# sleep3r/Diffusion-Handwriting-Generation.pytorch

Measured on AMD Instinct MI355X. Metric: stroke-points/sec reverse-sampled (T=60, L=488), higher is better.
Workload: dtype bf16; 1 GPU; configs[1]: batch=64 prompts/GPU, T=60, L=488, Lt=30, d_model=128/192/256, num_layers=2, diffusion_mode=new, random-init weights; global_batch=64, seq_len=488, parallelism=batch-shard x1 (no collectives)

## Files before the change

diffusion-handwriting-generation.pytorch_amd/build.py:

```python
from __future__ import annotations

import os
import subprocess
import sys
from concurrent.futures import ThreadPoolExecutor

HERE = os.path.dirname(os.path.abspath(__file__))
CSRC = os.path.join(HERE, "csrc")
LIB = os.path.join(HERE, "libdhw_hip.so")
SOURCES = ["train/sgemm_f32.hip", "train/sgemm_bf16.hip", "train/sgemm_group.hip", "convblock.hip", "ragged/convblock_ragged.hip", "enclayer.hip",
           "ragged/enclayer_ragged.hip", "policy/convblock_policy.hip", "policy/enclayer_policy.hip", "gemm.hip", "ragged/gemm_ragged.hip", "ragged/attn_ragged.hip", "persist.hip", "attn.hip", "misc.hip", "style.hip", "textside.hip",
           "train.hip", "train/sgemm_launch.hip", "train/elementwise.hip", "train/film_table.hip", "train/batch.hip", "render/render.hip", "cond/cond.hip", "score/score.hip", "attnmap/attnmap.hip",
           "dhw_api.cpp", "dhw_style_api.cpp", "dhw_train_api.cpp",
           "render/dhw_render_api.cpp", "cond/dhw_cond_api.cpp", "score/dhw_score_api.cpp", "attnmap/dhw_attnmap_api.cpp", "sampler/weights.cpp", "sampler/workspace.cpp", "sampler/denoiser.cpp", "sampler/sample.cpp", "sampler/debug.cpp",
           "step/step.hip", "step/dhw_step_api.cpp", "page/page.hip", "page/dhw_page_api.cpp", "encode/encode.hip", "encode/dhw_encode_api.cpp",
           "prep/prep.hip", "prep/dhw_prep_api.cpp", "train/cond_drop.hip"]
FLAGS = ["--offload-arch=gfx950", "-O3", "-fPIC", "-std=c++17", "-Wall", "-Wno-unused-function", "-Wno-unused-value", "-Wno-unused-result"]


def _hipcc() -> str:
    for c in (os.environ.get("HIPCC"), "/opt/rocm/bin/hipcc", "hipcc"):
        if c and (os.path.sep not in c or os.path.exists(c)):
            return c
    raise RuntimeError("hipcc not found")


def _stale(target: str, deps: list[str]) -> bool:
    if not os.path.exists(target):
        return True
    t = os.path.getmtime(target)
    return any(os.path.getmtime(d) > t for d in deps)


def _obj(objdir: str, s: str) -> str:
    return os.path.join(objdir, s.rsplit(".", 1)[0].replace("/", "_") + ".o")


def build(force: bool = False, verbose: bool = False) -> str:
    hipcc = _hipcc()
    headers = [os.path.join(d, f) for d, _, files in os.walk(CSRC) for f in files if f.endswith(".h")]
    headers += [os.path.join(HERE, "..", "include", f) for f in ("dhw.h", "dhw_debug.h", "dhw_style.h", "dhw_train.h")]
    objdir = os.path.join(HERE, "build")
    os.makedirs(objdir, exist_ok=True)
    jobs = []
# ... 29 lines not shown
```

diffusion-handwriting-generation.pytorch_amd/csrc/dhw_api.cpp:

```cpp
#include <algorithm>
#include <cstdarg>
#include <cstdlib>
#include <cstring>

#include "host/error.h"
#include "sampler/handle.h"
#include "xcd_swizzle.h"

static ErrBuf g_err;

void set_global_error(const char* fmt, va_list ap) noexcept { g_err.vsetf(fmt, ap); }

int fail(dhw_handle* h, int code, const char* fmt, ...) noexcept {
  va_list ap;
  va_start(ap, fmt);
  g_err.vsetf(fmt, ap);
  va_end(ap);
  if (h) h->err.set(g_err.c_str());
  return code;
}

extern "C" {

const char* dhw_version(void) { return "dhw-hip 0.1 (gfx950)"; }
// ... 40 lines not shown
    h->store.init(build_spec(d.num_layers, d.c1, d.c2, d.c3));
    h->pspec = build_spec(d.num_layers, d.c1, h->dims.c2, d.c3);
    build_film_layout(h);
    build_names(h);
    if (hipSetDevice(device) != hipSuccess) return fail(nullptr, DHW_ERR_HIP, "hipSetDevice failed");
    {
      const char* e = getenv("DHW_STREAMS");
      if (e && atoi(e) >= 1) h->nstreams = std::min(atoi(e), MAX_STREAMS);
      h->nstreams = std::max(1, std::min(h->nstreams, d.max_B));
      h->nstreams_alloc = h->nstreams;
    }
    int rc = alloc_shared(h);
    h->ws.resize(h->nstreams);
    for (int i = 0; !rc && i < h->nstreams; ++i)
      if (!(rc = alloc_workspace(h, h->ws[i], i == 0 ? d.max_B : (d.max_B + h->nstreams - 1) / h->nstreams))) rc = verify_workspace(h, h->ws[i]);
    for (int i = 1; !rc && i < h->nstreams; ++i)
      if (hipStreamCreateWithFlags(&h->sub_streams[i], hipStreamNonBlocking) != hipSuccess) rc = fail(h, DHW_ERR_HIP, "stream create failed");
    if (const char* e = getenv("DHW_FUSE")) h->fuse = atoi(e) != 0;
    if (const char* e = getenv("DHW_PLANE")) h->plane = atoi(e) != 0;
    if (const char* e = getenv("DHW_FUSE_TEXT")) h->fuse_text = atoi(e) != 0;
    if (const char* e = getenv("DHW_FUSE_HEADS")) h->fuse_heads = atoi(e) != 0;
    if (const char* e = getenv("DHW_FUSE_UP")) h->fuse_up = atoi(e) != 0;
    if (const char* e = getenv("DHW_CHAIN")) h->chain = atoi(e) != 0;
    if (const char* e = getenv("DHW_PERSIST")) h->persist = atoi(e) != 0;
    if (const char* e = getenv("DHW_PLANE_REUSE")) h->plane_reuse = atoi(e) != 0;
    if (const char* e = getenv("DHW_TEXT_PAIRS")) h->text_pairs = atoi(e) == 1 ? 1 : atoi(e) == 2 ? 2 : 0;
    if (const char* e = getenv("DHW_STORE_POLICY")) {
      const long v = strtol(e, nullptr, 0);
      bool ok = v >= 0 && v < 64;
      for (int cls = 0; ok && cls < 3; ++cls) ok = store_policy_of((int)v, cls) != 3;
      if (!ok && !rc) rc = fail(h, DHW_ERR_ARG, "DHW_STORE_POLICY=%s: two bits per output class (C, A, B from bit 0), each 0 = plain, 1 = write-through, 2 = early release", e);
      if (ok) h->store_policy = (int)v;
    }
    if (!rc && h->store_policy != DHW_STORE_DEFAULT && (enclayer_init_policy() != hipSuccess || convblock_init_policy() != hipSuccess))
      rc = fail(h, DHW_ERR_HIP, "kernel attribute setup failed: %s", hipGetErrorString(hipGetLastError()));
    if (h->padded) h->fuse = false;
    if (!rc && h->prec == PREC_BF16 && h->persist) {
      hipDeviceProp_t prop;
      if (hipGetDeviceProperties(&prop, device) != hipSuccess || persist_init() != hipSuccess) rc = fail(h, DHW_ERR_HIP, "persistent kernel setup failed: %s", hipGetErrorString(hipGetLastError()));
      else {
        h->persist_grid = prop.multiProcessorCount;
        if (hipHostMalloc((void**)&h->h_step_err, 64, hipHostMallocMapped) != hipSuccess || hipHostGetDevicePointer((void**)&h->d_step_err, h->h_step_err, 0) != hipSuccess)
          rc = fail(h, DHW_ERR_HIP, "host-mapped error word: %s", hipGetErrorString(hipGetLastError()));
        else *h->h_step_err = 0;
      }
    }
    if (!rc && enclayer_init() != hipSuccess) rc = fail(h, DHW_ERR_HIP, "kernel attribute setup failed: %s", hipGetErrorString(hipGetLastError()));
    if (!rc && (enclayer_init_ragged() != hipSuccess || convblock_init_ragged() != hipSuccess || gemm_init_ragged() != hipSuccess))
      rc = fail(h, DHW_ERR_HIP, "kernel attribute setup failed: %s", hipGetErrorString(hipGetLastError()));
    if (!rc && convblock_init() != hipSuccess) rc = fail(h, DHW_ERR_HIP, "kernel attribute setup failed: %s", hipGetErrorString(hipGetLastError()));
    if (!rc && textside_init() != hipSuccess) rc = fail(h, DHW_ERR_HIP, "kernel attribute setup failed: %s", hipGetErrorString(hipGetLastError()));
    if (!rc && gemm_init() != hipSuccess) rc = fail(h, DHW_ERR_HIP, "kernel attribute setup failed: %s", hipGetErrorString(hipGetLastError()));
    if (rc) { ErrBuf keep = h->err; g_err = keep; return rc; }
    hold.p = nullptr;
    *out = h;
    return 0;
  });
}

void dhw_destroy(dhw_handle* h) {
  if (!h) return;
  try {
    destroy_impl(h);
  } catch (...) {
  }
}

// ... 123 lines not shown
```

diffusion-handwriting-generation.pytorch_amd/csrc/dhw_kernels.h:

```cpp
#pragma once
#include <hip/hip_runtime.h>
#include <stdint.h>

enum { PREC_BF16 = 0, PREC_F32 = 1 };

#define DHW_LENS_DEV __host__ __device__
#ifndef DHW_LENS
#define DHW_LENS 0
#endif

enum { STORE_PLAIN = 0, STORE_WT = 1, STORE_EARLY = 2 };
constexpr int store_policy_of(int word, int cls) { return (word >> (2 * cls)) & 3; }
#define DHW_STORE_DEFAULT 21
#ifdef DHW_STORE_RT
#define DHW_STORE_OF(field, cls) (field)
#else
#ifndef DHW_STORE_FIXED
#define DHW_STORE_FIXED DHW_STORE_DEFAULT
#endif
#define DHW_STORE_OF(field, cls) store_policy_of(DHW_STORE_FIXED, cls)
#endif

struct GemmSeg {
  const void* A;
  const void* W;
  int C;
  int taps;
  int silu;
};

struct GemmParams {
  GemmSeg seg[2];
  int nseg;
  int B, L;
  int N;
  int n_store;
  const float* bias0;
  const float* bias1;
  const float* posb;
  int posb_cols;
  const float* gam;
  const float* bet;
  long film_bs;
  int film_div;
  int film_mode;
  const void* res1;
  const void* res2;
  int res2_half;
  int ln;
  int ln_n;
  float ln_inv;
  int silu_out;
  int relu6_out;
// ... 67 lines not shown
  const float *b_q1, *b_d1, *b_qkv2, *b_d2, *b_f1, *b_f2;
  const float *pb_q1, *pb_qk2;
  const float* film; long film_bs; int film_tot; int f1, f2, f3;
  const void* k1; const void* vt1; int lpadT;
  const int64_t* text;
  void* x2;
  void* qk2; void* vt2; int lpadX;
  void* out; void* pool;
  int bm_min;
  int dbg;
  unsigned long long* stamps;
  const int* lens; int lsh;
  int store_a, store_bc;
};
struct EncChain {
  int mode;
  EncLayerParams a;
  const void* w_dense; const float* b_dense;
  void* dense_out;
};
bool convblock_chain_supported(int prec, const ConvBlockParams& p, const EncChain& chain);
hipError_t launch_convblock_chain(int prec, const ConvBlockParams& p, const EncChain& chain, hipStream_t st);
hipError_t launch_convblock_chain_ragged(int prec, const ConvBlockParams& p, const EncChain& chain, hipStream_t st);
hipError_t launch_convblock_chain_policy(int prec, const ConvBlockParams& p, const EncChain& chain, hipStream_t st);
bool convblock_chain_auto(const ConvBlockParams& p);
bool enclayer_supported(int prec, int d, int heads);
bool enclayer_chain_supported(int prec, int d, int B, int Lk, int mode, int d_next);
hipError_t launch_enclayer(int prec, const EncLayerParams& p, int which, hipStream_t st, const EncChain* chain = nullptr);
hipError_t enclayer_init();
hipError_t launch_enclayer_ragged(int prec, const EncLayerParams& p, int which, hipStream_t st, const EncChain* chain);
hipError_t enclayer_init_ragged();
hipError_t launch_enclayer_policy(int prec, const EncLayerParams& p, int which, hipStream_t st, const EncChain* chain);
hipError_t enclayer_init_policy();

struct AttnParams {
  const void* Q; int ldq;
  const void* K; int ldk; int koff;
  const void* Vt; int lpad;
  const int64_t* text; int ldt;
  void* out; int ldo;
  int B, H, D, Lq, Lk;
  const int* lens; int lsh;
  int lens_keys;
};
hipError_t launch_attn(int prec, const AttnParams& p, hipStream_t st);
hipError_t launch_attn_ragged(int prec, const AttnParams& p, hipStream_t st);

hipError_t launch_sigma_ffn(const float* sigma, int n, const float* w1, const float* b1,
                            const float* w2, const float* b2, float* sig32, hipStream_t st);
hipError_t launch_film(const float* sig32, int n, const float* wcat, const float* bcat, int cols,
                       float* film, hipStream_t st);
hipError_t launch_embed_ln(int prec, const int64_t* text, int rows, const float* emb, int dim, int n_true, int vocab,
                           void* out, hipStream_t st);
hipError_t launch_film_apply(int prec, const void* in, int in_B, int B, int rows, int dim, const float* gam,
                             const float* bet, long bs, int div, void* out, hipStream_t st);
hipError_t launch_cast(int prec, const float* in, long n, void* out, hipStream_t st);
hipError_t launch_input_dense(int prec, const float* strokes, long rows, const float* w, const float* b,
                              int C, void* out, hipStream_t st);

hipError_t launch_heads(const HeadsParams& p, hipStream_t st);
hipError_t launch_randn_init(float* xt, long rows, int L, const uint64_t* seed_ptr, int sample_off, hipStream_t st, int iter = -1);
hipError_t launch_set_seed(uint64_t* seed_ptr, uint64_t seed, int64_t first_sample, hipStream_t st, unsigned* plane_skip = nullptr,
                           unsigned host_ok = 0);
hipError_t launch_stage_compare(const void* text, void* text_stage, size_t text_bytes, const void* style, void* style_stage, size_t style_bytes,
                                unsigned* plane_skip, hipStream_t st);
hipError_t launch_zero_tail(float* x, int B, int L, int C, const int* lens, hipStream_t st);
// ... 91 lines not shown
```

diffusion-handwriting-generation.pytorch_amd/csrc/enc_bc_core.h:

```cpp
#pragma once
#include "enc_a_core.h"

namespace {

#define STAMP(slot) ENC_STAMP(slot)
#ifdef DHW_STAMPS
#define WST(slot) do { if (p.stamps && blockIdx.x == 0 && lane == 0) p.stamps[64 + wave * 32 + (slot)] = __builtin_amdgcn_s_memtime(); } while (0)
#else
#define WST(slot) do { } while (0)
#endif

template <typename T, int DM, int BM, typename P>
DHW_DEV void enc_a_tile(const P& p, const int b, const int m0, char* smem) {
  const int S = tile_stride<T>(DM);
  EncALds m;
  m.XR = smem;
  m.QR = m.XR + BM * S;
  m.red = reinterpret_cast<float*>(m.QR + BM * S);
  m.KT = reinterpret_cast<char*>(m.red) + 2 * 8 * BM * sizeof(float);
  m.VT = m.KT + 32 * tile_stride<T>(DM);
  m.VS = smem;
  m.PL = reinterpret_cast<float*>(m.KT + enc_a_text_kv_bytes<T, DM, BM>());
  const int Ls = sample_len(p.lens, p.lsh, b, p.Lk);
  if constexpr (DHW_LENS) { if (m0 >= Ls) return; }
// ... 53 lines not shown
  const float* gam = p.film + (size_t)b * p.film_bs;
  const float* bet = gam + p.film_tot;
  const int row0 = wm * (BM / WM), ntile0 = wn * NT;
  const int n0 = ntile0 * 16 + 4 * g;
  const size_t wlane = ((size_t)ntile0 * KC * 64 + lane) * 8;
  const char* op1 = R1 + (row0 + l15) * S + g * 8 * ES;
  const char* op3 = R3 + (row0 + l15) * S + g * 8 * ES;

  WRing<T, NT, RING, RDMAX> ring;
  constexpr bool SPREAD = sizeof(T) == 2;
  constexpr int FCH = WRing<T, NT, RING, RDMAX>::template fill_chunks<KC>(), FQ = (FCH + 3) / 4;
  EpiParams<NT> ep;
  constexpr bool PLDS = enc_plds<T>(), PLFIX = bc_params_fixed<T, DM, BM>();
  float* PL = reinterpret_cast<float*>(smem + lds_bc_tiles<T, DM, BM>());
  ParamStage<8> cp;
#define BC_PARAMS_REQUEST() cp.template load<DM>(tid, p.b_d2, gam + p.f2, bet + p.f2, p.b_f1, p.b_f1 + DM, p.b_f2, gam + p.f3, bet + p.f3)
  STAMP(16);
  WST(0);
  DHW_STAMP_IF(p.stamps && blockIdx.x == 0 && threadIdx.x == 0, 40, __builtin_amdgcn_s_memtime());
  if (!(p.dbg & 1)) {
    constexpr int RG = BM / 16, HS = 8 / RG, UMAX = (H + HS - 1) / HS, KBS = self_kbs<T, DM, BM>();
    constexpr bool DB = self_db<T, DM, BM>();
    constexpr bool VROW = sizeof(T) == 2;
    constexpr int SK = tile_stride<T>(DM), SV = VROW ? SK : KBS * ES + self_vpad<T, DM, BM>();
    constexpr int BUFB = KBS * SK + (VROW ? KBS * SV : DM * SV);
    constexpr int QKS = qkv_stride<T, DM>();
    const int rg = wave % RG, hs = wave / RG;
    auto unit_head = [&](int u) { return hs + u * HS; };
    const T* qk = reinterpret_cast<const T*>(p.qk2);
    const T* ksrc = qk + (size_t)b * p.Lk * QKS + DM;
    const T* vsrc = VROW ? ksrc + DM : reinterpret_cast<const T*>(p.vt2) + (size_t)b * DM * p.lpadX;
    constexpr int EPV = 16 / ES, CPR = DM / EPV, PPR = KBS / EPV;
    constexpr int UK = (KBS * CPR + 511) / 512, UV = VROW ? UK : (DM * PPR + 511) / 512;
    CopyRegs<UK> ck;
    CopyRegs<UV> cv;
    auto request = [&](int kb) {
      ck.load(KBS * CPR, tid, 512, [&](int id) { const int r = id / CPR, cc = id - r * CPR;
                                                 return reinterpret_cast<const uint4*>(ksrc + (size_t)min(kb + r, p.Lk - 1) * QKS + cc * EPV); });
      if constexpr (VROW)
        cv.load(KBS * CPR, tid, 512, [&](int id) { const int r = id / CPR, cc = id - r * CPR;
                                                   return reinterpret_cast<const uint4*>(vsrc + (size_t)min(kb + r, p.Lk - 1) * QKS + cc * EPV); });
      else
        cv.load(DM * PPR, tid, 512, [&](int id) { const int ch = id / PPR, part = id - ch * PPR;
                                                  return reinterpret_cast<const uint4*>(vsrc + (size_t)ch * p.lpadX + (kb + (part + 1) * EPV <= p.lpadX ? kb + part * EPV : 0)); });
    };
    auto commit = [&](int kb, char* KT, char* VT) {
      ck.store(KBS * CPR, tid, 512, [&](int id) { const int r = id / CPR, cc = id - r * CPR; return reinterpret_cast<uint4*>(KT + r * SK + cc * 16); },
               [&](int id) { return kb + id / CPR < Ls; });
      if constexpr (VROW)
        cv.store(KBS * CPR, tid, 512, [&](int id) { const int r = id / CPR, cc = id - r * CPR; return reinterpret_cast<uint4*>(VT + r * SV + cc * 16); },
                 [&](int id) { return kb + id / CPR < Ls; });
      else
        cv.store_to(DM * PPR, tid, 512, [&](int id, const uint4& v) { const int ch = id / PPR, part = id - ch * PPR; vt_store_piece<T>(VT + ch * SV, part, v); },
                    [&](int id) { return kb + (id % PPR + 1) * EPV <= p.lpadX && (!DHW_LENS || kb + (id % PPR) * EPV < Ls); });
    };
    Frag<T> qf[UMAX][2];
    float mr[UMAX], lr[UMAX];
    f32x4 o[UMAX][4];
#pragma unroll
    for (int u = 0; u < UMAX; ++u) {
      const int h = unit_head(u);
      const T* qrow = qk + (size_t)(b * p.Lk + m0 + rg * 16 + l15) * QKS + (h < H ? h : 0) * 64 + 8 * g;
      qf[u][0] = frag_load(qrow);
      qf[u][1] = frag_load(qrow + 32);
      mr[u] = -INFINITY;
      lr[u] = 0.f;
#pragma unroll
      for (int t = 0; t < 4; ++t) o[u][t] = (f32x4){0, 0, 0, 0};
    }
    if constexpr (PLDS) BC_PARAMS_REQUEST();
    request(0);
    if constexpr (PLDS && PLFIX) cp.template store<DM>(PL, tid);
    commit(0, R2, R2 + KBS * SK);
    lds_barrier();
    int ib = 0;
    auto key_block = [&](int kb) {
      const bool more = kb + KBS < Ls;
      char* KT = R2 + (DB && (ib & 1) ? BUFB : 0);
      char* VT = KT + KBS * SK;
      char* KN = R2 + (DB && !(ib & 1) ? BUFB : 0);
      if (DB && more) request(kb + KBS);
      if (ib < 3) STAMP(26 + 2 * ib);
      attn_units<T, KBS, false, UMAX>(lane, qf, KT, SK, VT, SV, hs, HS, H, kb, 0u, Ls, mr, lr, o);
      if (ib < 3) STAMP(27 + 2 * ib);
      if (more) {
        if (!DB) {
          lds_barrier();
          request(kb + KBS);
        }
        commit(kb + KBS, KN, KN + KBS * SK);
        lds_barrier();
      }
    };
    for (int kb = 0; kb < Ls; kb += KBS, ++ib) key_block(kb);
    if constexpr (PLDS && !PLFIX) {
      static_assert(DB, "a single staging buffer leaves room for a fixed parameter block");
      static_assert((size_t)2 * BM * tile_stride<T>(DM) + 2 * 8 * BM * sizeof(float) + enc_bc_param_bytes<T, DM>() <= (size_t)BUFB, "parameter block inside buffer 0");
      PL = reinterpret_cast<float*>(((ib - 1) & 1) ? R2 + 2 * BM * S + 2 * 8 * BM * sizeof(float) : R2 + BUFB);
      cp.template store<DM>(PL, tid);
    }
    WST(1);
#pragma unroll
    for (int u = 0; u < UMAX; ++u) {
      const int h = unit_head(u);
      float l = lr[u];
      l = xg_sum(l);
      const float inv = 1.0f / l;
      if (h < H) {
        T* dst = reinterpret_cast<T*>(R1 + (rg * 16 + l15) * S) + h * 64 + 4 * g;
        store_pair(lane, dst, dst + 16, o[u][0] * inv, o[u][1] * inv);
        store_pair(lane, dst + 32, dst + 48, o[u][2] * inv, o[u][3] * inv);
      }
    }
  }
  else if constexpr (PLDS) {
    BC_PARAMS_REQUEST();
    if constexpr (!PLFIX) PL = reinterpret_cast<float*>(R2 + 2 * BM * S + 2 * 8 * BM * sizeof(float));
    cp.template store<DM>(PL, tid);
  }
  if (act) {
    ring.template fill_s<KC>(reinterpret_cast<const T*>(p.w_d2) + wlane);
    if constexpr (!PLDS) ep.load(p.b_d2, gam + p.f2, bet + p.f2, n0);
  }
// ... 175 lines not shown
```

diffusion-handwriting-generation.pytorch_amd/csrc/gemm_core.h:

```cpp
#pragma once
#include "dhw_common.h"
#include "dhw_kernels.h"
#include "epilogue.h"

template <typename T> constexpr int OPAD = sizeof(T) == 2 ? 32 : 16;
template <typename T> __host__ __device__ constexpr int tile_stride(int C) { return C * (int)sizeof(T) + OPAD<T>; }

DHW_DEV void keep_alive(const Frag<bf16_t>& f) { asm volatile("" ::"v"(f.v)); }
DHW_DEV void keep_alive(const Frag<float>& f) { asm volatile("" ::"v"(f.lo), "v"(f.hi)); }

#ifndef DHW_ABL
#define DHW_ABL 0
#endif
template <typename T, int NT, int RING = (sizeof(T) == 2 ? 24 : 12), int DMAX = 8>
struct WRing {
  static constexpr int D0 = RING / NT;
  static constexpr int D = D0 < 2 ? 2 : (D0 > DMAX ? DMAX : D0);
  Frag<T> q[D][NT];
  const T* base;
  int KT, KTS;

  DHW_DEV void fill(const T* __restrict__ wbase, int kt, int kts = 0) {
    base = wbase;
    KT = kt;
    KTS = kts ? kts : kt;
#pragma unroll
    for (int d = 0; d < D; ++d) {
      const int k = d < KT ? d : KT - 1;
#pragma unroll
      for (int i = 0; i < NT; ++i) q[d][i] = frag_load(base + ((size_t)i * KTS + k) * 512);
    }
  }

  template <int MT, int ABL = DHW_ABL>
  DHW_DEV void run(f32x4 (&acc)[NT][MT], const char* abase, int stride, int KC) {
    constexpr int ES = sizeof(T);
// ... 182 lines not shown
#pragma unroll
      for (int e = 0; e < PER; ++e)
        if (KT_ + s * PER + e < DN) next_chunk(KT_ + s * PER + e);
      __builtin_amdgcn_sched_barrier(0);
    }
    base = nbase; KT = KTN_; KTS = nKTS;
  }
};

template <typename T, int MT, int NT, int RING = (sizeof(T) == 2 ? 24 : 12), int ABL = 0>
DHW_DEV void mainloop(f32x4 (&acc)[NT][MT], const T* __restrict__ wbase, const char* abase, int stride, int KC, int taps,
                      int KTS = 0) {
  WRing<T, NT, RING> ring;
  ring.fill(wbase, KC * taps, KTS);
  ring.template run<MT, ABL>(acc, abase, stride, KC);
}

DHW_DEV __amdgpu_buffer_rsrc_t tile_rsrc(const void* base, unsigned bytes) {
  const unsigned long long a = reinterpret_cast<unsigned long long>(base);
  const unsigned lo = __builtin_amdgcn_readfirstlane((unsigned)a), hi = __builtin_amdgcn_readfirstlane((unsigned)(a >> 32));
  return __builtin_amdgcn_make_buffer_rsrc(reinterpret_cast<void*>(((unsigned long long)hi << 32) | lo), 0, __builtin_amdgcn_readfirstlane(bytes), 0x00020000);
}
DHW_DEV void store16_wt(__amdgpu_buffer_rsrc_t rsrc, unsigned byte_off, const uint4& v) {
  typedef unsigned u32x4_t __attribute__((ext_vector_type(4)));
  __builtin_amdgcn_raw_buffer_store_b128((u32x4_t){v.x, v.y, v.z, v.w}, rsrc, byte_off, 0, 16);
}
DHW_DEV void tile_release_early(int tid) {
  asm volatile("s_waitcnt vmcnt(0)\n\ts_barrier" ::: "memory");
  if (tid == 0) {
    __builtin_amdgcn_fence(__ATOMIC_RELEASE, "agent");
    asm volatile("s_waitcnt vmcnt(0)" ::: "memory");
  }
}

template <typename T>
DHW_DEV void tile_copy_out(const char* lds, int S, T* gdst, int gs, int rows_valid, int C, int tid, int nthreads, int policy = STORE_PLAIN) {
  constexpr int ES = sizeof(T), EPV = 16 / ES;
  const int cpr = C / EPV;
  const int total = rows_valid * cpr;
  if (policy == STORE_WT) {
    if (total <= 0) return;
    const __amdgpu_buffer_rsrc_t rsrc = tile_rsrc(gdst, (unsigned)(((rows_valid - 1) * gs + C) * ES));
    for (int id = tid; id < total; id += nthreads) {
      const int r = id / cpr, cc = id - r * cpr;
      store16_wt(rsrc, (unsigned)((r * gs + cc * EPV) * ES), *reinterpret_cast<const uint4*>(lds + r * S + cc * 16));
    }
    return;
  }
  for (int id = tid; id < total; id += nthreads) {
    const int r = id / cpr, cc = id - r * cpr;
    *reinterpret_cast<uint4*>(gdst + (size_t)r * gs + cc * EPV) = *reinterpret_cast<const uint4*>(lds + r * S + cc * 16);
  }
}
template <typename T>
DHW_DEV void tile_copy_out_pool(const char* lds, int S, T* gdst, int gs, int rows_valid_in, int C, int tid, int nthreads, int policy = STORE_PLAIN) {
  constexpr int ES = sizeof(T), EPV = 16 / ES;
  const int cpr = C / EPV;
  const int total = (rows_valid_in / 2) * cpr;
  if (policy == STORE_WT) {
    if (total <= 0) return;
    const __amdgpu_buffer_rsrc_t rsrc = tile_rsrc(gdst, (unsigned)(((rows_valid_in / 2 - 1) * gs + C) * ES));
    for (int id = tid; id < total; id += nthreads) {
      const int r = id / cpr, cc = id - r * cpr;
      uint4 a = *reinterpret_cast<const uint4*>(lds + (2 * r) * S + cc * 16);
      const uint4 b = *reinterpret_cast<const uint4*>(lds + (2 * r + 1) * S + cc * 16);
      T* ea = reinterpret_cast<T*>(&a);
// ... 110 lines not shown
```

diffusion-handwriting-generation.pytorch_amd/csrc/policy/enclayer_policy.hip:

```cpp
#define DHW_STORE_RT 1
#define launch_enclayer launch_enclayer_policy
#define enclayer_supported enclayer_supported_policy
#define enclayer_chain_supported enclayer_chain_supported_policy
#define enclayer_init enclayer_init_policy
#include "../enclayer.hip"
```

diffusion-handwriting-generation.pytorch_amd/csrc/sampler/denoiser.cpp:

```cpp
#include <cstdlib>

#include "denoiser.h"

static int level_shift(int L_full, int L) {
  int k = 0;
  while ((L << k) < L_full) ++k;
  return k;
}

static void rec_phase(Ctx& c, int kind, int L, const ConvBlockParams* cb, const EncLayerParams* el, const EncChain* nx) {
  int rows = 0, lv = 0;
  if (!step_kind_geometry(kind, L, &rows, &lv) || (int)c.rec->size() >= STEP_MAX_PHASES) { c.rec_fail = true; return; }
  StepPhase ph{};
  ph.kind = kind;
  ph.rows = rows;
  ph.tps = (lv + rows - 1) / rows;
  if (cb) ph.cb = *cb;
  if (el) ph.el = *el;
  if (nx) ph.nx = *nx;
  c.rec->push_back(ph);
}

void* need(Ctx& c, void* p, const char* what) {
  if (!p && !c.err) c.err = fail(c.h, DHW_ERR_INTERNAL, "internal: workspace buffer '%s' was never allocated", what);
// ... 215 lines not shown
    vt1p += (size_t)c.plane_step * c.B * (v_rows(h, w) ? c.Lt : h->lpadT) * d * h->es;
  }
  EncLayerParams q{};
  q.B = c.B; q.Lk = Lk; q.Lt = c.Lt; q.d = d; q.heads = w.heads;
  q.x = x;
  q.w_q1 = w.w_q1; q.w_d1 = w.w_d1; q.w_qkv2 = w.w_qkv2; q.w_d2 = w.w_d2; q.w_f1 = w.w_f1; q.w_f2 = w.w_f2;
  q.b_q1 = w.b_q1; q.b_d1 = w.b_d1; q.b_qkv2 = w.b_qkv2; q.b_d2 = w.b_d2; q.b_f1 = w.b_f1; q.b_f2 = w.b_f2;
  q.pb_q1 = w.pb_q1; q.pb_qk2 = w.pb_qk2;
  q.film = c.film; q.film_bs = c.film_bs; q.film_tot = h->film_tot; q.f1 = w.f1; q.f2 = w.f2; q.f3 = w.f3;
  q.k1 = k1p; q.vt1 = vt1p; q.lpadT = h->lpadT; q.text = text;
  q.x2 = ELB(c, li, x2); q.qk2 = ELB(c, li, qk2); q.vt2 = ELB(c, li, vt2); q.lpadX = lpad;
  q.out = ELB(c, li, out); q.pool = pool;
  q.lens = c.lens; q.lsh = level_shift(c.L, Lk);
  q.store_a = store_policy_of(h->store_policy, 1); q.store_bc = store_policy_of(h->store_policy, 2);
  return q;
}

static void enc_layer(Ctx& c, int li, const EncLayerW& w, const void* x, int Lk, int lpad, const int64_t* text,
               void* pool, bool skip_a = false, const EncChain* chain = nullptr, int bm_min = 0) {
  dhw_handle* h = c.h;
  const int d = w.d;
  const char* k1p = (const char*)ELK(c, li, k1);
  const char* vt1p = (const char*)ELK(c, li, vt1);
  if (c.use_plane) {
    k1p += (size_t)c.plane_step * c.B * c.Lt * d * h->es;
    vt1p += (size_t)c.plane_step * c.B * (v_rows(h, w) ? c.Lt : h->lpadT) * d * h->es;
  }
  if (h->fuse && enclayer_supported(h->prec, d, w.heads)) {
    EncLayerParams q = enc_params(c, li, w, x, Lk, lpad, text, pool);
    q.bm_min = bm_min;
    const double rows = (double)c.B * Lk, dd = d;
    if (c.rec) {
      const bool chained = chain && chain->mode;
      if (h->prec != PREC_BF16) { c.rec_fail = true; return; }
      if (!skip_a) {
        if (d == 256) rec_phase(c, PK_A256, c.L, nullptr, &q, nullptr);
        else c.rec_fail = true;
      }
      int kind = -1;
      if (d == 192 && !chained && skip_a) kind = PK_BC192;
      else if (d == 256 && chained && chain->mode == 2 && !skip_a && bm_min == 32 && !(Lk & 1)) kind = PK_BC256_N2;
      else if (d == 384 && chained && chain->mode == 1 && skip_a) kind = PK_BC384_N1;
      else if (d == 384 && !chained && skip_a) kind = PK_BC384;
      if (kind < 0) { c.rec_fail = true; return; }
      rec_phase(c, kind, c.L, nullptr, &q, chained ? chain : nullptr);
      return;
    }
    for (int which = skip_a ? 1 : 0; which < 2 && !c.err; ++which) {
      double fl = which == 0 ? 2.0 * rows * dd * dd * 5 + 4.0 * rows * c.Lt * dd
                             : 2.0 * rows * dd * dd * 5 + 4.0 * rows * Lk * dd;
      double by = (which == 0 ? rows * dd * 5 : rows * dd * (5 + (pool ? 0.5 : 0.0))) * h->es + 5.0 * dd * dd * h->es;
      const EncChain* ch = which == 1 ? chain : nullptr;
      if (ch && ch->mode) {
        const double r2 = (double)c.B * ch->a.Lk, d2 = ch->a.d;
        fl += 2.0 * r2 * d2 * d2 * 5 + 4.0 * r2 * c.Lt * d2 + (ch->mode == 2 ? 2.0 * r2 * dd * d2 : 0.0);
        by += r2 * d2 * 5 * h->es + 5.0 * d2 * d2 * h->es;
      }
      Launch l(h, c.st, which == 0 ? "enc.fused_a" : (ch && ch->mode ? "enc.fused_bc+a" : "enc.fused_bc"), fl, by);
      hipError_t e = q.lens ? launch_enclayer_ragged(h->prec, q, which, c.st, ch)
                     : h->store_policy != DHW_STORE_DEFAULT ? launch_enclayer_policy(h->prec, q, which, c.st, ch) : launch_enclayer(h->prec, q, which, c.st, ch);
      if (e != hipSuccess) c.err = fail(h, DHW_ERR_HIP, "enclayer %s/%d: %s", h->el_name[li].c_str(), which, hipGetErrorString(e));
    }
    tap(c, tap_el(li, 1), ELB(c, li, x2), Lk, d);
    tap(c, tap_el(li, 0), ELB(c, li, out), Lk, d);
    return;
  }
  if (c.rec) { c.rec_fail = true; return; }
  {
    GemmParams p = gp_stroke(c, Lk, d);
    p.seg[0] = GemmSeg{x, w.w_q1, d, 1, 0};
    p.bias0 = w.b_q1;
    p.posb = w.pb_q1;
    p.posb_cols = d;
    p.out = ELB(c, li, q1);
    run_gemm(c, "enc.q_cross", p);
  }
  {
    AttnParams a{};
    a.Q = ELB(c, li, q1); a.ldq = d;
    a.K = k1p; a.ldk = d; a.koff = 0;
    a.Vt = vt1p; a.lpad = h->lpadT;
    a.text = text; a.ldt = c.Lt;
    a.out = ELB(c, li, a1); a.ldo = d;
    a.B = c.B; a.H = w.heads; a.D = d / w.heads; a.Lq = Lk; a.Lk = c.Lt;
    a.lens = c.lens; a.lsh = level_shift(c.L, Lk);
    run_attn(c, "attn.cross", a);
  }
  {
    GemmParams p = gp_stroke(c, Lk, d);
    p.seg[0] = GemmSeg{ELB(c, li, a1), w.w_d1, d, 1, 0};
    p.bias0 = w.b_d1;
    p.ln = 1;
    set_film(c, p, w.f1, 1);
// ... 287 lines not shown
```

diffusion-handwriting-generation.pytorch_amd/csrc/sampler/handle.h:

```cpp
#pragma once
#include <hip/hip_runtime.h>

#include <cstdint>
#include <map>
#include <string>
#include <vector>

#include "../../../include/dhw.h"
#include "../../../include/dhw_debug.h"
#include "../abi_guard.h"
#include "../dhw_kernels.h"
#include "../persist.h"
#include "plane_tag.h"
#include "../host/device_arena.h"
#include "../host/weight_store.h"

#pragma GCC visibility push(hidden)

constexpr int SIG = 32, SIG_HID = 2048, VOCAB = 73, STYLE_CH = 256;
constexpr int SLACK_ROWS = 64;

struct ProfRec { int label; hipEvent_t a, b; double flops, bytes; int plane_call = -1; };
struct ProfAgg { std::string label; double ms = 0, flops = 0, bytes = 0; int64_t n = 0; };

// ... 67 lines not shown

  float *sg_w1, *sg_b1, *sg_w2, *sg_b2, *in_w, *in_b, *out_w, *out_b, *pen_w, *pen_b, *emb;

  ConvBlockW enc1, enc2, enc4, dec3, dec2, dec1;
  std::vector<EncLayerW> el;
  void *w_sf1, *w_sf3, *w_q8, *w_kv8, *w_d8, *w_tf1, *w_tf3, *w_attd, *w_sk1, *w_sk2, *w_sk3;
  float *b_sf1, *b_sf3, *b_q8, *b_kv8, *b_d8, *b_tf1, *b_tf3, *b_attd, *b_sk1, *b_sk2, *b_sk3;
  int f_ts1, f_ts2, f_ts3, f_ts4;

  std::vector<Workspace> ws;
  int nstreams = 1;
  int nstreams_alloc = 1;
  hipStream_t sub_streams[MAX_STREAMS] = {};
  std::vector<TapSlot> taps;
  std::vector<std::string> el_name;
  int lpadT = 0, lpadS = 0, lpadX[3] = {0, 0, 0};

  bool prof = false;
  std::vector<std::string> prof_labels;
  std::vector<ProfRec> prof_recs;
  std::vector<ProfAgg> prof_agg;

  bool use_graph = true;
  int teach_every = 0;
  const float* teach_reset = nullptr;
  float* teach_capture = nullptr;
  bool fuse_heads = true;
  bool plane = true;
  bool fuse_up = true;
  bool chain = true;
  bool fuse = true;
  bool fuse_text = true;
  int store_policy = DHW_STORE_DEFAULT;
  int text_pairs = 0;
  std::map<std::vector<uint64_t>, hipGraphExec_t> graphs;
  std::map<std::vector<uint64_t>, uint64_t> graph_plane_gen;
  int64_t* d_text_stage = nullptr;
  float* d_style_stage = nullptr;
  float* d_out_stage = nullptr;
  float* d_noise_stage = nullptr;
  size_t noise_stage_cap = 0;
  float* d_known_stage = nullptr;
  unsigned char* d_keep_stage = nullptr;
  float* d_cond_noise_stage = nullptr;
  size_t cond_noise_stage_cap = 0;
  struct DenoiseScratch { float *x = nullptr, *w = nullptr, *eps = nullptr, *pen = nullptr, *sigma = nullptr; } scratch;
  uint64_t* d_seed = nullptr;
  bool plane_reuse = true;
  PlaneTag plane_tag;
  uint64_t weights_gen = 0, plane_gen = 0;
  unsigned* d_plane_skip = nullptr;
  long plane_calls = 0;
  unsigned* h_prof_skip = nullptr;
  int prof_calls = 0;
  static constexpr int PROF_SKIP_CAP = 4096;
  int* d_lens = nullptr;
  int* h_lens_pin = nullptr;
  hipEvent_t lens_ev = nullptr;
  float* d_guide_scale = nullptr;
  float* h_guide_scale_pin = nullptr;
  hipEvent_t guide_ev = nullptr;

  bool persist = false;
  int persist_grid = 0;
  unsigned* d_step_sync = nullptr;
  size_t step_sync_words = 0;
// ... 81 lines not shown
```

diffusion-handwriting-generation.pytorch_amd/csrc/sampler/sample.cpp:

```cpp
#include <algorithm>
#include <cmath>
#include <cstdlib>
#include <cstring>

#include "../cond/cond.h"
#include "denoiser.h"

int check_shapes(dhw_handle* h, int B, int L, int Lt, const char* fn) {
  const dhw_dims& d = h->dims;
  if (B < 1 || B > d.max_B || L < 8 || L > d.max_L || L % 8 || Lt < 1 || Lt > d.max_Lt)
    return fail(h, DHW_ERR_ARG, "%s%sshape out of range: B=%d (max %d) L=%d (max %d, multiple of 8) Lt=%d (max %d)", fn ? fn : "", fn ? ": " : "",
                B, d.max_B, L, d.max_L, Lt, d.max_Lt);
  return 0;
}

static int ensure_film_T(dhw_handle* h, int T, dhw_handle::FilmT** out) {
  dhw_handle::FilmT& ft = h->film_T[T];
  *out = &ft;
  if (ft.d_film) return 0;
  int rc;
  if ((rc = dev_alloc(h, (void**)&ft.d_sigma, (size_t)T * 4))) return rc;
  if ((rc = dev_alloc(h, (void**)&ft.d_sig32, (size_t)T * SIG * 4))) return rc;
  if ((rc = dev_alloc(h, (void**)&ft.d_film, (size_t)T * 2 * h->film_tot * 4))) return rc;
  return 0;
// ... 339 lines not shown
      hipDeviceSynchronize();
      drop_graphs(h);
      if (h->d_step_sync) hipMemset(h->d_step_sync, 0, h->step_sync_words * sizeof(unsigned));
      if (code >= 0x100u)
        return fail(h, DHW_ERR_HIP, "persistent step kernel: XCD %u owns samples but no workgroup of the launch ran there in an EARLIER call (partitioned / "
                    "CU-masked device?): those samples were never computed; persistent launches are now disabled for this handle", code - 0x100u);
      return fail(h, DHW_ERR_HIP, "persistent step kernel timed out waiting for phase %u in an EARLIER call (its samples were invalid); "
                  "persistent launches are now disabled for this handle", code - 1);
    }
    dhw_handle::FilmT* ft = nullptr;
    if ((rc = ensure_film_T(h, T, &ft))) return rc;
    h->d_film_T = ft->d_film;
    if (h->plane) {
      const int ns = std::min(h->nstreams, B), per = (B + ns - 1) / ns;
      for (int s = 0; s < ns; ++s)
        if ((rc = ensure_plane(h, h->ws[s], plane_chunk(T), per))) return rc;
    }
    std::vector<float> beta, alpha;
    schedule_host(T, beta, alpha);
    if (!ft->ready) {
      ft->h_sigma.resize(T);
      for (int i = 0; i < T; ++i) ft->h_sigma[i] = sqrtf(alpha[i]);
      HIPCK(h, hipMemcpyAsync(ft->d_sigma, ft->h_sigma.data(), T * 4, hipMemcpyHostToDevice, st));
      Ctx c{h, &h->ws[0], st, B, L, Lt, h->dims.S * 5, ft->d_film, 0};
      RUN_SMALL(c, "sigma_ffn", launch_sigma_ffn(ft->d_sigma, T, h->sg_w1, h->sg_b1, h->sg_w2, h->sg_b2, ft->d_sig32, st));
      RUN_SMALL(c, "film_table", launch_film(ft->d_sig32, T, h->d_film_w, h->d_film_b, 2 * h->film_tot, ft->d_film, st));
      if (c.err) return c.err;
      ft->ready = true;
    }
    const size_t rows = (size_t)B * L;
    if (noise && (rc = grow_stage(h, &h->d_noise_stage, &h->noise_stage_cap, (size_t)(T + 1) * rows * 2))) return rc;
    if (cond && cond->cond_noise && (rc = grow_stage(h, &h->d_cond_noise_stage, &h->cond_noise_stage_cap, (size_t)T * rows * 2))) return rc;
    const bool graph = h->use_graph && !h->prof && !h->teach_every;
    const std::vector<uint64_t> key = {(uint64_t)B, (uint64_t)L, (uint64_t)Lt, (uint64_t)T, (uint64_t)mode, (uint64_t)(noise != nullptr), (uint64_t)h->nstreams, (uint64_t)h->plane, (uint64_t)h->fuse_heads, (uint64_t)h->fuse_up, (uint64_t)h->chain, (uint64_t)h->persist, (uint64_t)h->store_policy,
                                         (uint64_t)ragged,
                                         (uint64_t)(cond != nullptr), (uint64_t)(cond ? cond->t_start : T), (uint64_t)(cond && cond->keep), (uint64_t)(cond && cond->cond_noise)};
    PlaneTag call_tag;
    {
      auto gen = h->graph_plane_gen.find(key);
      call_tag.valid = true;
      call_tag.B = B; call_tag.nstreams = h->nstreams; call_tag.Lt = Lt; call_tag.S = h->dims.S; call_tag.T = T;
      call_tag.t_start = cond ? cond->t_start : T;
      call_tag.weights_gen = h->weights_gen;
      call_tag.film = ft->d_film;
      call_tag.plane_gen = graph && gen != h->graph_plane_gen.end() ? gen->second : h->plane_gen;
    }
    const PlaneGate gate{h->plane_reuse, h->plane, h->fuse && h->fuse_text && textside_supported(h->prec, Lt, h->dims.S * 5, 2 * h->dims.c2)};
    const unsigned host_ok = plane_host_ok(h->plane_tag, call_tag, gate);
    plane_invalidate(h);
    {
      hipError_t e = launch_set_seed(h->d_seed, seed, first_sample, st, h->d_plane_skip, host_ok);
      if (e != hipSuccess) return fail(h, DHW_ERR_HIP, "set_seed: %s", hipGetErrorString(e));
    }

    {
      hipError_t e = launch_stage_compare(text, h->d_text_stage, (size_t)B * Lt * 8, style, h->d_style_stage, (size_t)B * h->dims.S * 1280 * 4, h->d_plane_skip, st);
      if (e != hipSuccess) return fail(h, DHW_ERR_HIP, "stage_compare: %s", hipGetErrorString(e));
    }
    int plane_call = -1;
    if (h->prof && h->h_prof_skip && h->prof_calls < dhw_handle::PROF_SKIP_CAP) {
      plane_call = h->prof_calls++;
      HIPCK(h, hipMemcpyAsync(h->h_prof_skip + plane_call, h->d_plane_skip, 4, hipMemcpyDeviceToHost, st));
    }
    const float* nz = nullptr;
    if (noise) {
      const size_t need = (size_t)(T + 1) * rows * 2;
      if ((rc = grow_stage(h, &h->d_noise_stage, &h->noise_stage_cap, need))) return rc;
// ... 98 lines not shown
```

Before: 1.840 million stroke-points/s.

## Stage attention K/V tiles into LDS via buffer_load direct-to-LDS DMA

In the bf16 encoder-layer attention core, K and V tile staging now uses buffer_load ... lds instructions that write global data straight into LDS with out-of-range reads returning zero. This replaces the register round-trip (load to VGPRs, then store to LDS), which is meant to cut VGPR pressure and store instructions in the key-block loop. The old register path is kept as separate policy/ragged variants selected by DHW_STAGE_DMA=0, and the graph cache key now includes the flag. The risks are inline-asm m0 handling, the exactness of the LDS offset layout, and a full vmcnt(0) wait that may also serialize other outstanding loads.

```diff
diff --git a/diffusion-handwriting-generation.pytorch_amd/build.py b/diffusion-handwriting-generation.pytorch_amd/build.py
--- a/diffusion-handwriting-generation.pytorch_amd/build.py
+++ b/diffusion-handwriting-generation.pytorch_amd/build.py
@@ -9,7 +9,7 @@
 CSRC = os.path.join(HERE, "csrc")
 LIB = os.path.join(HERE, "libdhw_hip.so")
 SOURCES = ["train/sgemm_f32.hip", "train/sgemm_bf16.hip", "train/sgemm_group.hip", "convblock.hip", "ragged/convblock_ragged.hip", "enclayer.hip",
-           "ragged/enclayer_ragged.hip", "policy/convblock_policy.hip", "policy/enclayer_policy.hip", "gemm.hip", "ragged/gemm_ragged.hip", "ragged/attn_ragged.hip", "persist.hip", "attn.hip", "misc.hip", "style.hip", "textside.hip",
+           "ragged/enclayer_ragged.hip", "policy/convblock_policy.hip", "policy/enclayer_policy.hip", "policy/enclayer_ragged_policy.hip", "gemm.hip", "ragged/gemm_ragged.hip", "ragged/attn_ragged.hip", "persist.hip", "attn.hip", "misc.hip", "style.hip", "textside.hip",
            "train.hip", "train/sgemm_launch.hip", "train/elementwise.hip", "train/film_table.hip", "train/batch.hip", "render/render.hip", "cond/cond.hip", "score/score.hip", "attnmap/attnmap.hip",
            "dhw_api.cpp", "dhw_style_api.cpp", "dhw_train_api.cpp",
            "render/dhw_render_api.cpp", "cond/dhw_cond_api.cpp", "score/dhw_score_api.cpp", "attnmap/dhw_attnmap_api.cpp", "sampler/weights.cpp", "sampler/workspace.cpp", "sampler/denoiser.cpp", "sampler/sample.cpp", "sampler/debug.cpp",
diff --git a/diffusion-handwriting-generation.pytorch_amd/csrc/dhw_api.cpp b/diffusion-handwriting-generation.pytorch_amd/csrc/dhw_api.cpp
--- a/diffusion-handwriting-generation.pytorch_amd/csrc/dhw_api.cpp
+++ b/diffusion-handwriting-generation.pytorch_amd/csrc/dhw_api.cpp
@@ -96,7 +96,10 @@
       if (!ok && !rc) rc = fail(h, DHW_ERR_ARG, "DHW_STORE_POLICY=%s: two bits per output class (C, A, B from bit 0), each 0 = plain, 1 = write-through, 2 = early release", e);
       if (ok) h->store_policy = (int)v;
     }
+    if (const char* e = getenv("DHW_STAGE_DMA")) h->stage_dma = atoi(e) != 0;
     if (!rc && h->store_policy != DHW_STORE_DEFAULT && (enclayer_init_policy() != hipSuccess || convblock_init_policy() != hipSuccess))
+      rc = fail(h, DHW_ERR_HIP, "kernel attribute setup failed: %s", hipGetErrorString(hipGetLastError()));
+    if (!rc && !h->stage_dma && (enclayer_init_policy() != hipSuccess || enclayer_init_ragged_regs() != hipSuccess))
       rc = fail(h, DHW_ERR_HIP, "kernel attribute setup failed: %s", hipGetErrorString(hipGetLastError()));
     if (h->padded) h->fuse = false;
     if (!rc && h->prec == PREC_BF16 && h->persist) {
diff --git a/diffusion-handwriting-generation.pytorch_amd/csrc/dhw_kernels.h b/diffusion-handwriting-generation.pytorch_amd/csrc/dhw_kernels.h
--- a/diffusion-handwriting-generation.pytorch_amd/csrc/dhw_kernels.h
+++ b/diffusion-handwriting-generation.pytorch_amd/csrc/dhw_kernels.h
@@ -19,6 +19,10 @@
 #define DHW_STORE_FIXED DHW_STORE_DEFAULT
 #endif
 #define DHW_STORE_OF(field, cls) store_policy_of(DHW_STORE_FIXED, cls)
+#endif
+
+#ifndef DHW_STAGE_REGS
+#define DHW_STAGE_REGS 0
 #endif
 
 struct GemmSeg {
@@ -152,6 +156,8 @@
 hipError_t enclayer_init_ragged();
 hipError_t launch_enclayer_policy(int prec, const EncLayerParams& p, int which, hipStream_t st, const EncChain* chain);
 hipError_t enclayer_init_policy();
+hipError_t launch_enclayer_ragged_regs(int prec, const EncLayerParams& p, int which, hipStream_t st, const EncChain* chain);
+hipError_t enclayer_init_ragged_regs();
 
 struct AttnParams {
   const void* Q; int ldq;
diff --git a/diffusion-handwriting-generation.pytorch_amd/csrc/enc_bc_core.h b/diffusion-handwriting-generation.pytorch_amd/csrc/enc_bc_core.h
--- a/diffusion-handwriting-generation.pytorch_amd/csrc/enc_bc_core.h
+++ b/diffusion-handwriting-generation.pytorch_amd/csrc/enc_bc_core.h
@@ -109,8 +109,16 @@
     const T* vsrc = VROW ? ksrc + DM : reinterpret_cast<const T*>(p.vt2) + (size_t)b * DM * p.lpadX;
     constexpr int EPV = 16 / ES, CPR = DM / EPV, PPR = KBS / EPV;
     constexpr int UK = (KBS * CPR + 511) / 512, UV = VROW ? UK : (DM * PPR + 511) / 512;
-    CopyRegs<UK> ck;
-    CopyRegs<UV> cv;
+    constexpr bool SDMA = sizeof(T) == 2 && !DHW_STAGE_REGS;
+    const int wave_u = __builtin_amdgcn_readfirstlane(wave);
+    TileDma<KBS, SK, DM * ES, QKS * ES> dma;
+    if constexpr (SDMA) dma.init(wave_u, lane);
+    auto stage = [&](int kb, char* KT) {
+      dma.request(ksrc + (size_t)kb * QKS, Ls - kb, KT, wave_u);
+      dma.request(vsrc + (size_t)kb * QKS, Ls - kb, KT + KBS * SK, wave_u);
+    };
+    CopyRegs<SDMA ? 1 : UK> ck;
+    CopyRegs<SDMA ? 1 : UV> cv;
     auto request = [&](int kb) {
       ck.load(KBS * CPR, tid, 512, [&](int id) { const int r = id / CPR, cc = id - r * CPR;
                                                  return reinterpret_cast<const uint4*>(ksrc + (size_t)min(kb + r, p.Lk - 1) * QKS + cc * EPV); });
@@ -146,9 +154,16 @@
       for (int t = 0; t < 4; ++t) o[u][t] = (f32x4){0, 0, 0, 0};
     }
     if constexpr (PLDS) BC_PARAMS_REQUEST();
-    request(0);
+    if constexpr (SDMA) stage(0, R2);
+    else request(0);
     if constexpr (PLDS && PLFIX) cp.template store<DM>(PL, tid);
-    commit(0, R2, R2 + KBS * SK);
+    if constexpr (SDMA) {
+      tile_dma_wait();
+#pragma unroll
+      for (int u = 0; u < UMAX; ++u) { keep_alive(qf[u][0]); keep_alive(qf[u][1]); }
+      if constexpr (PLDS) asm volatile("" ::"v"(cp.v0.x), "v"(cp.v1.x));
+    }
+    else commit(0, R2, R2 + KBS * SK);
     lds_barrier();
     int ib = 0;
     auto key_block = [&](int kb) {
@@ -156,16 +171,17 @@
       char* KT = R2 + (DB && (ib & 1) ? BUFB : 0);
       char* VT = KT + KBS * SK;
       char* KN = R2 + (DB && !(ib & 1) ? BUFB : 0);
-      if (DB && more) request(kb + KBS);
+      if (DB && more) { if constexpr (SDMA) stage(kb + KBS, KN); else request(kb + KBS); }
       if (ib < 3) STAMP(26 + 2 * ib);
       attn_units<T, KBS, false, UMAX>(lane, qf, KT, SK, VT, SV, hs, HS, H, kb, 0u, Ls, mr, lr, o);
       if (ib < 3) STAMP(27 + 2 * ib);
       if (more) {
         if (!DB) {
           lds_barrier();
-          request(kb + KBS);
+          if constexpr (SDMA) stage(kb + KBS, KN); else request(kb + KBS);
         }
-        commit(kb + KBS, KN, KN + KBS * SK);
+        if constexpr (SDMA) tile_dma_wait();
+        else commit(kb + KBS, KN, KN + KBS * SK);
         lds_barrier();
       }
     };
diff --git a/diffusion-handwriting-generation.pytorch_amd/csrc/gemm_core.h b/diffusion-handwriting-generation.pytorch_amd/csrc/gemm_core.h
--- a/diffusion-handwriting-generation.pytorch_amd/csrc/gemm_core.h
+++ b/diffusion-handwriting-generation.pytorch_amd/csrc/gemm_core.h
@@ -2,6 +2,7 @@
 #include "dhw_common.h"
 #include "dhw_kernels.h"
 #include "epilogue.h"
+#include "host/tile_image.h"
 
 template <typename T> constexpr int OPAD = sizeof(T) == 2 ? 32 : 16;
 template <typename T> __host__ __device__ constexpr int tile_stride(int C) { return C * (int)sizeof(T) + OPAD<T>; }
@@ -250,6 +251,37 @@
     asm volatile("s_waitcnt vmcnt(0)" ::: "memory");
   }
 }
+
+template <int ROWS, int S, int DATA, int SRB>
+struct TileDma {
+  static constexpr int NP = tile_dma_pieces(ROWS, S), U = (NP + 7) / 8;
+  uint32_t off[U];
+  DHW_DEV void init(int wave, int lane) {
+    static_assert(ROWS * S % TILE_DMA_PIECE == 0 && S % TILE_DMA_LANE == 0 && DATA % TILE_DMA_LANE == 0 && DATA <= S && DATA <= SRB, "whole pieces, no lane across a boundary");
+#pragma unroll
+    for (int u = 0; u < U; ++u) {
+      const int p = wave + 8 * u;
+      off[u] = tile_dma_offset((p < NP ? p : 0) * TILE_DMA_PIECE + TILE_DMA_LANE * lane, S, DATA, SRB);
+    }
+  }
+  DHW_DEV void request(const void* src, int rows_left, char* lds, int wave) const {
+    typedef unsigned u32x4_t __attribute__((ext_vector_type(4)));
+    const unsigned long long a = reinterpret_cast<unsigned long long>(src);
+    const u32x4_t rsrc = {(unsigned)__builtin_amdgcn_readfirstlane((unsigned)a), (unsigned)__builtin_amdgcn_readfirstlane((unsigned)(a >> 32)) & 0xffffu,
+                          (unsigned)__builtin_amdgcn_readfirstlane(tile_dma_records(rows_left, DATA, SRB)), 0x00020000u};
+    const unsigned l0 = __builtin_amdgcn_readfirstlane((unsigned)reinterpret_cast<size_t>(lds));
+#pragma unroll
+    for (int u = 0; u < U; ++u) {
+      const int p = wave + 8 * u;
+      if (8 * u + 7 < NP || p < NP) {
+        unsigned keep;
+        asm volatile("s_nop 4\n\ts_mov_b32 %0, m0\n\ts_mov_b32 m0, %1\n\ts_nop 0\n\tbuffer_load_dwordx4 %2, %3, 0 offen lds\n\ts_mov_b32 m0, %0"
+                     : "=&s"(keep) : "s"(l0 + (unsigned)p * TILE_DMA_PIECE), "v"(off[u]), "s"(rsrc) : "memory");
+      }
+    }
+  }
+};
+DHW_DEV void tile_dma_wait() { asm volatile("s_waitcnt vmcnt(0)" ::: "memory"); }
 
 template <typename T>
 DHW_DEV void tile_copy_out(const char* lds, int S, T* gdst, int gs, int rows_valid, int C, int tid, int nthreads, int policy = STORE_PLAIN) {
diff --git a/diffusion-handwriting-generation.pytorch_amd/csrc/host/tile_image.h b/diffusion-handwriting-generation.pytorch_amd/csrc/host/tile_image.h
--- /dev/null
+++ b/diffusion-handwriting-generation.pytorch_amd/csrc/host/tile_image.h
@@ -0,0 +1,29 @@
+#pragma once
+#include <cstdint>
+
+#if defined(__HIPCC__) || defined(__CUDACC__)
+#define DHW_TILE_HD __host__ __device__
+#else
+#define DHW_TILE_HD
+#endif
+
+constexpr uint32_t TILE_DMA_ZERO = 0x80000000u;
+constexpr int TILE_DMA_PIECE = 1024, TILE_DMA_LANE = 16;
+
+struct TileImageSrc { int row, col; bool data; };
+
+DHW_TILE_HD constexpr TileImageSrc tile_image_src(int o, int S, int data_bytes) { return TileImageSrc{o / S, o % S, o % S < data_bytes}; }
+
+DHW_TILE_HD constexpr uint32_t tile_dma_offset(int o, int S, int data_bytes, int src_row_bytes) {
+  return o % S < data_bytes ? (uint32_t)(o / S) * (uint32_t)src_row_bytes + (uint32_t)(o % S) : TILE_DMA_ZERO;
+}
+
+DHW_TILE_HD constexpr int tile_dma_pieces(int rows, int S) { return (rows * S + TILE_DMA_PIECE - 1) / TILE_DMA_PIECE; }
+
+DHW_TILE_HD constexpr uint32_t tile_dma_records(int rows_left, int data_bytes, int src_row_bytes) {
+  return (uint32_t)(rows_left - 1) * (uint32_t)src_row_bytes + (uint32_t)data_bytes;
+}
+
+DHW_TILE_HD constexpr bool tile_dma_reads_zero(uint32_t offset, uint32_t records, uint32_t size = TILE_DMA_LANE) {
+  return (uint64_t)offset + size > records;
+}
diff --git a/diffusion-handwriting-generation.pytorch_amd/csrc/policy/enclayer_policy.hip b/diffusion-handwriting-generation.pytorch_amd/csrc/policy/enclayer_policy.hip
--- a/diffusion-handwriting-generation.pytorch_amd/csrc/policy/enclayer_policy.hip
+++ b/diffusion-handwriting-generation.pytorch_amd/csrc/policy/enclayer_policy.hip
@@ -1,4 +1,5 @@
 #define DHW_STORE_RT 1
+#define DHW_STAGE_REGS 1
 #define launch_enclayer launch_enclayer_policy
 #define enclayer_supported enclayer_supported_policy
 #define enclayer_chain_supported enclayer_chain_supported_policy
diff --git a/diffusion-handwriting-generation.pytorch_amd/csrc/policy/enclayer_ragged_policy.hip b/diffusion-handwriting-generation.pytorch_amd/csrc/policy/enclayer_ragged_policy.hip
--- /dev/null
+++ b/diffusion-handwriting-generation.pytorch_amd/csrc/policy/enclayer_ragged_policy.hip
@@ -0,0 +1,8 @@
+#define DHW_LENS 1
+#define DHW_STORE_RT 1
+#define DHW_STAGE_REGS 1
+#define launch_enclayer launch_enclayer_ragged_regs
+#define enclayer_supported enclayer_supported_ragged_regs
+#define enclayer_chain_supported enclayer_chain_supported_ragged_regs
+#define enclayer_init enclayer_init_ragged_regs
+#include "../enclayer.hip"
diff --git a/diffusion-handwriting-generation.pytorch_amd/csrc/sampler/denoiser.cpp b/diffusion-handwriting-generation.pytorch_amd/csrc/sampler/denoiser.cpp
--- a/diffusion-handwriting-generation.pytorch_amd/csrc/sampler/denoiser.cpp
+++ b/diffusion-handwriting-generation.pytorch_amd/csrc/sampler/denoiser.cpp
@@ -271,7 +271,7 @@
     const double rows = (double)c.B * Lk, dd = d;
     if (c.rec) {
       const bool chained = chain && chain->mode;
-      if (h->prec != PREC_BF16) { c.rec_fail = true; return; }
+      if (h->prec != PREC_BF16 || !h->stage_dma) { c.rec_fail = true; return; }
       if (!skip_a) {
         if (d == 256) rec_phase(c, PK_A256, c.L, nullptr, &q, nullptr);
         else c.rec_fail = true;
@@ -296,8 +296,8 @@
         by += r2 * d2 * 5 * h->es + 5.0 * d2 * d2 * h->es;
       }
       Launch l(h, c.st, which == 0 ? "enc.fused_a" : (ch && ch->mode ? "enc.fused_bc+a" : "enc.fused_bc"), fl, by);
-      hipError_t e = q.lens ? launch_enclayer_ragged(h->prec, q, which, c.st, ch)
-                     : h->store_policy != DHW_STORE_DEFAULT ? launch_enclayer_policy(h->prec, q, which, c.st, ch) : launch_enclayer(h->prec, q, which, c.st, ch);
+      hipError_t e = q.lens ? (h->stage_dma ? launch_enclayer_ragged(h->prec, q, which, c.st, ch) : launch_enclayer_ragged_regs(h->prec, q, which, c.st, ch))
+                     : h->store_policy != DHW_STORE_DEFAULT || !h->stage_dma ? launch_enclayer_policy(h->prec, q, which, c.st, ch) : launch_enclayer(h->prec, q, which, c.st, ch);
       if (e != hipSuccess) c.err = fail(h, DHW_ERR_HIP, "enclayer %s/%d: %s", h->el_name[li].c_str(), which, hipGetErrorString(e));
     }
     tap(c, tap_el(li, 1), ELB(c, li, x2), Lk, d);
diff --git a/diffusion-handwriting-generation.pytorch_amd/csrc/sampler/handle.h b/diffusion-handwriting-generation.pytorch_amd/csrc/sampler/handle.h
--- a/diffusion-handwriting-generation.pytorch_amd/csrc/sampler/handle.h
+++ b/diffusion-handwriting-generation.pytorch_amd/csrc/sampler/handle.h
@@ -123,6 +123,7 @@
   bool fuse = true;
   bool fuse_text = true;
   int store_policy = DHW_STORE_DEFAULT;
+  bool stage_dma = true;
   int text_pairs = 0;
   std::map<std::vector<uint64_t>, hipGraphExec_t> graphs;
   std::map<std::vector<uint64_t>, uint64_t> graph_plane_gen;
diff --git a/diffusion-handwriting-generation.pytorch_amd/csrc/sampler/sample.cpp b/diffusion-handwriting-generation.pytorch_amd/csrc/sampler/sample.cpp
--- a/diffusion-handwriting-generation.pytorch_amd/csrc/sampler/sample.cpp
+++ b/diffusion-handwriting-generation.pytorch_amd/csrc/sampler/sample.cpp
@@ -395,7 +395,7 @@
     if (noise && (rc = grow_stage(h, &h->d_noise_stage, &h->noise_stage_cap, (size_t)(T + 1) * rows * 2))) return rc;
     if (cond && cond->cond_noise && (rc = grow_stage(h, &h->d_cond_noise_stage, &h->cond_noise_stage_cap, (size_t)T * rows * 2))) return rc;
     const bool graph = h->use_graph && !h->prof && !h->teach_every;
-    const std::vector<uint64_t> key = {(uint64_t)B, (uint64_t)L, (uint64_t)Lt, (uint64_t)T, (uint64_t)mode, (uint64_t)(noise != nullptr), (uint64_t)h->nstreams, (uint64_t)h->plane, (uint64_t)h->fuse_heads, (uint64_t)h->fuse_up, (uint64_t)h->chain, (uint64_t)h->persist, (uint64_t)h->store_policy,
+    const std::vector<uint64_t> key = {(uint64_t)B, (uint64_t)L, (uint64_t)Lt, (uint64_t)T, (uint64_t)mode, (uint64_t)(noise != nullptr), (uint64_t)h->nstreams, (uint64_t)h->plane, (uint64_t)h->fuse_heads, (uint64_t)h->fuse_up, (uint64_t)h->chain, (uint64_t)h->persist, (uint64_t)h->store_policy, (uint64_t)h->stage_dma,
                                          (uint64_t)ragged,
                                          (uint64_t)(cond != nullptr), (uint64_t)(cond ? cond->t_start : T), (uint64_t)(cond && cond->keep), (uint64_t)(cond && cond->cond_noise)};
     PlaneTag call_tag;
```

Result: no change. 1.848 million stroke-points/s (median of 6 runs) (+0.5%).
